# talmolab/sleap

Measured on NVIDIA H100. Metric: frames/sec (1024x1024 bottom-up UNet+PAF), higher is better.
Workload: dtype f16

## Files before the change

### sleap_b200/csrc/sb_conv_tc.cu

```cuda
#include <cuda.h>

#include <algorithm>

#include "sb_model.h"

namespace {

constexpr int TW = 16, TH = 8;
constexpr int MAX_GROUPS = 7, MAX_TAPS = 7;
constexpr size_t kMaxDynSmem = 225 * 1024;

struct TcTap { int row_off, w_tap; };
struct TcGroup { int dx, n_taps; TcTap taps[MAX_TAPS]; };

struct TcParams {
  int H, W;
  int tiles_x;
  int n_chunks, KC;
  int n_groups;
  TcGroup groups[MAX_GROUPS];
  int dy0, box_rows;
  int N, Cout;
  void* out;
  int out_f32, out_H, out_W, out_Ctot, out_coff;
// ... 689 lines not shown
    for (int bk = 0; bk < NB; ++bk) wgmma_reg_fence(acc[bk]);
    wgmma_wait<0>();
#pragma unroll
    for (int bk = 0; bk < NB; ++bk) wgmma_reg_fence(acc[bk]);
    __syncwarp();
    if (lane == 0) mbar_arrive(smem_u32(empty + s));

    const int tile = w % n_tiles, b = w / n_tiles;
    const int x0 = (tile % tiles_x) * 16, y0 = (tile / tiles_x) * (8 * BY);
#pragma unroll
    for (int bk = 0; bk < NB; ++bk)
      halo_block_epilogue<N>(P, acc[bk], smem_u32(s_bias), 0, b, y0 + 8 * (bk >> 1) + 2 * q, x0 + 8 * (bk & 1) + g, g, t, lo);
  }
}

constexpr int kWideThreads = 384;
constexpr int kWidePatchLoaders = 96;
constexpr int wide_by(int n) { return n <= 64 ? 4 : 2; }
constexpr int wide_plane(int n) { return (8 * wide_by(n) + 2) * kHaloCols * 16; }

template <int N>
__global__ void __launch_bounds__(kWideThreads, 1) k_conv_wg_hw(const __grid_constant__ CUtensorMap mapA,
                                                                const __grid_constant__ CUtensorMap mapB,
                                                                const __grid_constant__ TcParams P) {
  constexpr int BY = wide_by(N), NP = 8, PH = 8 * BY + 2, PW = kHaloCols, PLANE = wide_plane(N), SLOT = NP * PLANE;
  constexpr int WSLOT = N * 128;
  extern __shared__ __align__(1024) uint8_t smem_raw[];
  uint8_t* base = reinterpret_cast<uint8_t*>((reinterpret_cast<uintptr_t>(smem_raw) + 1023) & ~(uintptr_t)1023);
  uint8_t* wring = base;
  uint8_t* pring = wring + (size_t)P.n_b_slots * WSLOT;
// ... 419 lines not shown
  int threads;
  size_t smem;
  int max_ctas;
  int n_items;
  TcParams P;
  CUtensorMap mapA, mapB;
  TcPhases Q;
};

struct TcLaunch {
  dim3 grid;
  TcForm forms[kForms];
  int form;
};

}

struct SbConvTcPlan {
  std::vector<TcLaunch> launches;
  const void* head = nullptr;
  __half* w16 = nullptr;
  int Cout_pad = 0;
  bool pool_fused = false;
  bool out_dead = false;
  bool res_fused = false;
  std::vector<TcLaunch> plain_launches;
};

static CUtensorMapSwizzle swz_for(int KC) {
  return KC == 64 ? CU_TENSOR_MAP_SWIZZLE_128B : (KC == 32 ? CU_TENSOR_MAP_SWIZZLE_64B : CU_TENSOR_MAP_SWIZZLE_32B);
}

static bool tc_eligible(const SbModel* m, const SbOp& op) {
  if (getenv("SB_DISABLE_TC")) return false;
  if (op.kind() != SB_OPK_CONV && op.kind() != SB_OPK_TCONV) return false;
  const int Cin = op.in_C();
  if (!(Cin >= 16 && Cin % 8 == 0)) return false;
  if (op.kind() == SB_OPK_CONV && !((op.k() == 1 || op.k() == 3 || op.k() == 5 || op.k() == 7) && op.stride() == 1) &&
      !(op.k() == 1 && op.stride() == 2))
    return false;
  if (op.kind() == SB_OPK_CONV && op.explicit_pad() && (op.k() != 1 || op.pad_top() != 0 || op.pad_left() != 0)) return false;
// ... 135 lines not shown
  }
  F.n_items = P.n_tiles;
  fit_ctas(h, F, 1);
}

static bool res_fusable(const SbModel* m, size_t oi) {
  const SbOp& op = m->ops[oi];
  if (op.kind() != SB_OPK_CONV || !op.residual() || oi + 1 >= m->ops.size() || getenv("SB_DISABLE_RES_FUSION")) return false;
  const SbOp& add = m->ops[oi + 1];
  if (add.kind() != SB_OPK_ADD || !(add.flags() & SB_OPF_FUSED_ADD) || add.out_buf() != op.sum_buf() || add.out_coff() != op.sum_coff()) return false;
  const SbBuffer& rb = m->buffers[op.res_buf()];
  const SbBuffer& sb = m->buffers[op.sum_buf()];
  const SbBuffer& ob = m->buffers[op.out_buf()];
  return !rb.f32 && !sb.f32 && !ob.f32 && rb.C % 8 == 0 && op.res_coff() % 8 == 0 && sb.C % 8 == 0 && op.sum_coff() % 8 == 0 &&
         rb.H == ob.H && rb.W == ob.W && sb.H == ob.H && sb.W == ob.W && op.pool_buf() < 0 && !(op.flags() & (SB_OPF_BN | SB_OPF_RELU));
}

static CUresult encode_weights(EncodeTiledFn enc, const SbConvTcPlan* plan, int Cin, int n_wtaps, int KC, int box_n, CUtensorMap* map) {
  cuuint64_t dims[3] = {(cuuint64_t)Cin, (cuuint64_t)plan->Cout_pad, (cuuint64_t)n_wtaps};
  cuuint64_t strides[2] = {(cuuint64_t)Cin * 2, (cuuint64_t)plan->Cout_pad * Cin * 2};
  cuuint32_t box[3] = {(cuuint32_t)KC, (cuuint32_t)box_n, 1};
  cuuint32_t es[3] = {1, 1, 1};
  return enc(map, CU_TENSOR_MAP_DATA_TYPE_FLOAT16, 3, (void*)plan->w16, dims, strides, box, es, CU_TENSOR_MAP_INTERLEAVE_NONE,
             swz_for(KC), CU_TENSOR_MAP_L2_PROMOTION_L2_256B, CU_TENSOR_MAP_FLOAT_OOB_FILL_NONE);
}

static int make_launch(sb_handle_s* h, SbModel* m, const SbOp& op, SbConvTcPlan* plan, int n_groups,
                       const TcGroup* groups, int dy0, int extra_rows, int n_wtaps, int oy_mul, int oy_add,
                       int ox_mul, int ox_add, const SbTcView* view = nullptr, bool fuse_res = false,
                       std::vector<TcLaunch>* dst = nullptr) {
// ... 193 lines not shown
  }
#undef SB_HEAD_CASE
}

int sb_conv_tc_prepare(sb_handle_s* h, SbModel* m) {
  m->tc_plans.assign(m->ops.size(), nullptr);
  if (m->precision == 1) return 0;
  const bool split = m->precision == 2;
  static bool attr_set = false;
  if (!attr_set) {
    for (int f = 0; f < kForms; ++f)
      for (int kc : {16, 32, 64})
        for (int n : kWgN)
          if (const void* k = form_kernel(f, kc, n))
            SB_CUDA(h, cudaFuncSetAttribute(k, cudaFuncAttributeMaxDynamicSharedMemorySize, (int)kMaxDynSmem));
    attr_set = true;
  }
  for (size_t oi = 0; oi < m->ops.size(); ++oi) {
    const SbOp& op = m->ops[oi];
    if (!tc_eligible(m, op)) continue;
    const int Cin = op.in_C(), Cout = op.out_C(), k = op.k(), taps = k * k;
    SbConvTcPlan* plan = new SbConvTcPlan();
    int cp = (Cout + 15) / 16 * 16;
    if (cp > 256) cp = (cp + 255) / 256 * 256;
    plan->Cout_pad = cp;
    std::vector<__half> w16((size_t)taps * cp * Cin, __float2half(0.f));
    const float* w = m->weights_host.data() + op.w_off();
    for (int t = 0; t < taps; ++t)
      for (int ci = 0; ci < Cin; ++ci)
        for (int co = 0; co < Cout; ++co)
// ... 100 lines not shown
  TcParams P = F.P;
  P.skip_out = skip_out;
  dim3 grid(std::min(F.n_items * B, F.max_ctas));
  size_t smem = F.smem;
  if (L.form == 0) {
    grid = dim3(L.grid.x, L.grid.y, B);
    P.pdl_trigger = (sb_pdl_on() && smem >= 114 * 1024) ? 1 : 0;
    if (P.pdl_trigger) smem = std::max(smem, kMaxDynSmem);
  } else {
    P.batch = B;
  }
  void* args[4] = {const_cast<CUtensorMap*>(&F.mapA), const_cast<CUtensorMap*>(&F.mapB), &P, const_cast<TcPhases*>(&F.Q)};
  sb_launch_pdl(form_kernel(L.form, P.KC, P.N), grid, dim3(F.threads), smem, stream, args);
}

static int tc_launch(sb_handle_s* h, const std::vector<TcLaunch>& launches, int B, int skip_out) {
  for (const TcLaunch& L : launches) {
    launch_form(L, B, h->stream, skip_out);
    SB_CHECK_LAUNCH(h);
    if (L.form == kTconvForm) break;
  }
  return 0;
}

int sb_time_min(sb_handle_s* h, const char* what, float& best, const std::function<int()>& run) {
  cudaEvent_t e0, e1;
  SB_CUDA(h, cudaEventCreate(&e0));
  SB_CUDA(h, cudaEventCreate(&e1));
  best = 1e30f;
  int rc = 0;
// ... 51 lines not shown
    SbConvTcPlan* plan = m->tc_plans[oi];
    if (!plan || plan->launches.empty() || !plan->launches[0].forms[kTconvForm].ok) continue;
    TcLaunch& L0 = plan->launches[0];
    const int phase_form = L0.form;
    float best[2];
    for (int f = 0; f < 2; ++f) {
      L0.form = f ? kTconvForm : phase_form;
      snprintf(what, sizeof what, "op %zu, %s", oi, f ? "fused tconv" : "tconv phases");
      if (const int rc = sb_time_min(h, what, best[f], [&] { return tc_launch(h, plan->launches, m->B, 0); })) return rc;
    }
    L0.form = (force >= 0 ? force == kTconvForm : best[1] < best[0]) ? kTconvForm : phase_form;
    if (dbg)
      fprintf(stderr, "[sb_conv_tc] op %zu launches (4 tconv phases) %.1f us, fused k_tconv_wg_hw %.1f us -> %s\n", oi, best[0] * 1e3f,
              best[1] * 1e3f, L0.form == kTconvForm ? "tconv-fused" : "phases");
  }
  return 0;
}

static SbLaunchFn head_entry(const SbModel* m, const SbOp& op, const SbConvTcPlan* plan, bool log) {
  const SbBuffer& ib = m->buffers[op.in_buf()];
  const SbBuffer& ob = m->buffers[op.out_buf()];
  const HeadShape hs = head_shape(op);
  if (log && getenv("SB_DEBUG"))
    fprintf(stderr, "[sb_conv_tc] head k_head_1x1: Cin %d Cout %d NT %d KCH %d n_ring %d smem %zu\n", op.in_C(), op.out_C(), hs.nt,
            hs.kch, hs.n_ring, hs.smem);
  const void* kern = plan->head;
  const __half* in = (const __half*)ib.dev;
  const __half* w = plan->w16;
  const float* bias = op.b_off() >= 0 ? m->weights_dev + op.b_off() : nullptr;
  float* out = (float*)ob.dev;
  int in_Ctot = ib.C, in_coff = op.in_coff(), Cin = op.in_C(), out_Ctot = ob.C, out_coff = op.out_coff(), Cout = op.out_C();
  int relu = (op.flags() & SB_OPF_RELU) ? 1 : 0, n_ring = hs.n_ring;
  const size_t frame_pix = (size_t)ob.H * ob.W;
  return [=](sb_handle_s* h, const void*, int, int B) mutable {
    size_t npix = (size_t)B * frame_pix;
    void* args[] = {&in, &in_Ctot, &in_coff, &Cin, &w, &bias, &out, &out_Ctot, &out_coff, &Cout, &relu, &npix, &n_ring};
    const int grid = (int)std::min<size_t>((npix + 127) / 128, (size_t)h->sm_count * 2);
    sb_launch_pdl(kern, dim3(grid), dim3(256), hs.smem, h->stream, args);
    SB_CHECK_LAUNCH(h);
    return 0;
  };
}

SbTcEntry sb_conv_tc_entry(const SbModel* m, int op_index, bool all_stores) {
  const SbConvTcPlan* plan = m->tc_plans[op_index];
  SbTcEntry e;
  if (plan->head) {
    e.run = head_entry(m, m->ops[op_index], plan, !all_stores);
    return e;
  }
  const bool res = plan->res_fused && !all_stores;
  const int skip = plan->out_dead && !all_stores;
  const std::vector<TcLaunch>* launches = plan->res_fused && all_stores ? &plan->plain_launches : &plan->launches;
  e.run = [launches, skip](sb_handle_s* h, const void*, int, int B) { return tc_launch(h, *launches, B, skip); };
  if (plan->pool_fused || res) e.absorbs = op_index + 1;
  e.elides_out = skip || res;
  return e;
}
```

### sleap_b200/csrc/sb_entry.cu

```cuda
#include <algorithm>

#include "sb_model.h"

template <typename TI, int CIN, int COUT, int PX>
__global__ void __launch_bounds__(256) k_conv_first(const TI* __restrict__ img, int Hin, int Win, int Hnet, int Wnet,
                                                    __half* __restrict__ out, int out_Ctot, int out_coff,
                                                    const float* __restrict__ w ,
                                                    const float* __restrict__ bias, int relu, int in_is_u8, int split = 0) {
  __shared__ __align__(16) float s_w[9 * CIN * COUT];
  __shared__ float s_b[COUT];
  for (int t = threadIdx.y * 32 + threadIdx.x; t < 9 * CIN * COUT; t += 256) s_w[t] = w[t];
  for (int t = threadIdx.y * 32 + threadIdx.x; t < COUT; t += 256) s_b[t] = bias ? bias[t] : 0.f;
  __syncthreads();
  const int ox0 = (blockIdx.x * 32 + threadIdx.x) * PX, oy = blockIdx.y * 8 + threadIdx.y, b = blockIdx.z;
  if (ox0 >= Wnet || oy >= Hnet) return;
  const TI* im = img + (size_t)b * Hin * Win * CIN;
  const float sc = in_is_u8 ? (1.0f / 255.0f) : 1.0f;
  float acc[PX][COUT];
#pragma unroll
  for (int p = 0; p < PX; ++p)
#pragma unroll
    for (int c = 0; c < COUT; ++c) acc[p][c] = s_b[c];
#pragma unroll
  for (int ky = 0; ky < 3; ++ky) {
// ... 173 lines not shown
  if (cv.in_C() != ib.C || !only_reader(m, pre.out_buf(), p + 1)) return false;
  if (ib.H % 2 || ib.W % 2 || ob.H != ib.H / 2 || ob.W != ib.W / 2) return false;
  return !ob.f32 && ob.C % 8 == 0 && cv.out_coff() % 8 == 0;
}

bool conv01_fusable(const SbModel* m, int c0i) {
  if (m->precision != 0 || c0i + 1 >= (int)m->ops.size()) return false;
  const SbOp& c0 = m->ops[c0i];
  const SbOp& c1 = m->ops[c0i + 1];
  if (m->Cin != 1 || c0.in_C() != 1 || c0.out_C() != 16 || c0.k() != 3 || c0.stride() != 1 || (c0.flags() & SB_OPF_BN)) return false;
  if (c1.kind() != SB_OPK_CONV || c1.in_C() != 16 || c1.out_C() != 16 || c1.k() != 3 || c1.stride() != 1 || (c1.flags() & SB_OPF_BN)) return false;
  if (c1.in_buf() != c0.out_buf() || c1.in_coff() != c0.out_coff() || c1.pool_buf() < 0) return false;
  const SbBuffer& ob0 = m->buffers[c0.out_buf()];
  const SbBuffer& pb = m->buffers[c1.pool_buf()];
  if (ob0.f32 || pb.f32 || pb.C % 2 || c1.pool_coff() % 2 || ob0.H % 2 || ob0.W % 2) return false;
  return m->tc_plans[c0i + 1] && sb_conv_tc_entry(m, c0i + 1, false).elides_out && only_reader(m, c0.out_buf(), c0i + 1);
}


void free_view(SbEntryPlan& e) {
  if (e.view) cudaFree(e.view);
  if (e.view_bias) cudaFree(e.view_bias);
  e.view = nullptr;
  e.view_bias = nullptr;
}

int view_prepare(sb_handle_s* h, SbModel* m, int route, SbTcView& V, const std::vector<float>& w) {
  SbEntryPlan& e = m->entry;
  const size_t bytes = (size_t)m->B * e.view_H * e.view_W * 16 * sizeof(__half) + 256;
  SB_CUDA(h, cudaMalloc((void**)&e.view, bytes));
  SB_CUDA(h, cudaMemset(e.view, 0, bytes));
// ... 92 lines not shown
    } else {
      if (Cin == 1) launch_first<float, 1>(co, B, s, (const float*)frames_dev, Hin, Win, ob.H, ob.W, (__half*)ob.dev, ob.C, coff, Wt, bias, relu, 0, split);
      else launch_first<float, 3>(co, B, s, (const float*)frames_dev, Hin, Win, ob.H, ob.W, (__half*)ob.dev, ob.C, coff, Wt, bias, relu, 0, split);
    }
    SB_CHECK_LAUNCH(h);
    return 0;
  };
}

SbLaunchFn view_entry(SbModel* m) {
  const SbEntryPlan& e = m->entry;
  const int route = e.route, view_H = e.view_H, view_W = e.view_W, pre_mode = e.pre_mode;
  const int Cin = m->Cin, Hin = m->Hin, Win = m->Win;
  __half* view = e.view;
  const SbBuffer ib = m->buffers[m->ops[e.conv_op].in_buf()];
  const SbLaunchFn gemm = sb_conv_tc_entry(m, e.conv_op, false).run;
  return [=](sb_handle_s* h, const void* frames_dev, int frames_are_u8, int B) {
    const size_t total = (size_t)B * view_H * view_W;
    const int grid = (int)std::min<size_t>((total + 255) / 256, (size_t)h->sm_count * 16);
    cudaStream_t s = h->stream;
    if (route == SB_ENTRY_BUFFER_VIEW) {
      k_first_view<__half><<<grid, 256, 0, s>>>((const __half*)ib.dev, ib.H, ib.W, view_H, view_W, view, 0, total);
    } else if (route == SB_ENTRY_STEM_VIEW) {
      if (frames_are_u8)
        k_s2d_view<unsigned char><<<grid, 256, 0, s>>>((const unsigned char*)frames_dev, Hin, Win, Cin, view_H, view_W, view, 1,
                                                       total, pre_mode);
      else
        k_s2d_view<float><<<grid, 256, 0, s>>>((const float*)frames_dev, Hin, Win, Cin, view_H, view_W, view, 0, total, pre_mode);
    } else if (frames_are_u8) {
      k_first_view<unsigned char><<<grid, 256, 0, s>>>((const unsigned char*)frames_dev, Hin, Win, view_H, view_W, view, 1, total);
    } else {
// ... 50 lines not shown
      snprintf(what, sizeof what, "first layer, form %d", f);
      const int rc = sb_time_min(h, what, best[f], [&] { return cand[f](h, m->frames_dev, 1, m->B); });
      if (rc) return rc;
    }
    bool view = best[1] < best[0];
    if (const char* fv = getenv("SB_FORCE_FIRST_VIEW")) view = atoi(fv) != 0;
    if (dbg) fprintf(stderr, "[sb_conv_tc] op %d first layer: k_conv_first %.1f us, Toeplitz view + wgmma %.1f us -> %s\n", e.conv_op,
                     best[0] * 1e3f, best[1] * 1e3f, view ? "view" : "direct");
    if (!view) {
      sb_conv_tc_drop(m, e.conv_op);
      free_view(e);
      e.route = SB_ENTRY_DIRECT;
    }
  }
  if (e.conv01) {
    const SbLaunchFn conv0 = first_conv_entry(m), conv1 = sb_conv_tc_entry(m, e.conv_op + 1, false).run, fused_block = conv01_entry(e.conv01);
    float best[2];
    for (int f = 0; f < 2; ++f) {
      snprintf(what, sizeof what, "first block, fused %d", f);
      const int rc = sb_time_min(h, what, best[f], [&] {
        if (f == 1) return fused_block(h, m->frames_dev, 1, m->B);
        const int rc0 = conv0(h, m->frames_dev, 1, m->B);
        return rc0 ? rc0 : conv1(h, m->frames_dev, 1, m->B);
      });
      if (rc) return rc;
    }
    bool fused = best[1] < best[0];
    if (const char* fv = getenv("SB_FORCE_CONV01")) fused = atoi(fv) != 0;
    if (dbg) fprintf(stderr, "[sb_conv_tc] first block (B = %d): conv0 + conv1 launches %.1f us, fused k_conv01 %.1f us -> %s\n", m->B,
                     best[0] * 1e3f, best[1] * 1e3f, fused ? "fused" : "separate");
    if (fused) e.conv1_op = e.conv_op + 1;
  }
  return 0;
}

void sb_entry_build(SbModel* m, bool all_stores, std::vector<char>& taken) {
  const SbEntryPlan& e = m->entry;
  if (e.pre_op >= 0) taken[e.pre_op] = 1;
  if (e.conv_op < 0) return;
  const bool fused = e.conv1_op >= 0 && !all_stores;
  m->prog[all_stores][e.conv_op] = fused ? conv01_entry(e.conv01) : first_conv_entry(m);
  taken[e.conv_op] = 1;
  if (fused) taken[e.conv1_op] = taken[e.conv1_op + 1] = 1;
  if (e.conv01) m->buf_elided[m->ops[e.conv_op].out_buf()] = m->buf_elided[m->ops[e.conv_op + 1].out_buf()] = 1;
}

void sb_entry_release(SbModel* m) {
  free_view(m->entry);
  sb_conv01_release(m);
  m->entry = SbEntryPlan();
}
```

### sleap_b200/csrc/sb_model.cu

```cuda
#include <algorithm>

#include "sb_common.cuh"
#include "sb_kernels_direct.cuh"
#include "sb_model.h"

using namespace sbd;

namespace {

template <typename T> T* buf_ptr(const SbBuffer& b) { return (T*)b.dev; }

size_t elem_size(const SbModel* m, const SbBuffer& b) { return (b.f32 || m->precision == 1) ? 4 : 2; }

int grid_for(size_t total, int sm) {
  size_t g = (total + 255) / 256;
  size_t cap = (size_t)sm * 16;
  return (int)std::max<size_t>(1, std::min(g, cap));
}

int build_programs(sb_handle_s* h, SbModel* m);

}

void sb_models_free(sb_handle_s* h) {
// ... 297 lines not shown
    case SB_OPK_COPY:
      slot = [=](sb_handle_s* h, const void*, int, int B) {
        const size_t npix = (size_t)B * ob.H * ob.W;
        k_copy<T><<<grid_for(npix * op.in_C(), h->sm_count), 256, 0, h->stream>>>((const T*)ib.dev, ib.C, op.in_coff(), (T*)ob.dev, ob.C,
                                                                                  op.out_coff(), op.in_C(), npix);
        SB_CHECK_LAUNCH(h);
        return 0;
      };
      return 0;
    default:
      return sb_fail(h, SB_ERR_INVALID, "unknown op kind %d", op.kind());
  }
}

int build_programs(sb_handle_s* h, SbModel* m) {
  const size_t n = m->ops.size();
  m->op_kind.assign(n, 0);
  for (size_t oi = 0; oi < n; ++oi)
    if (m->ops[oi].kind() == SB_OPK_CONV || m->ops[oi].kind() == SB_OPK_TCONV) m->op_kind[oi] = m->tc_plans[oi] ? 1 : 2;
  m->buf_elided.assign(m->buffers.size(), 0);
  for (int all_stores = 0; all_stores < 2; ++all_stores) {
    m->prog[all_stores].assign(n, nullptr);
    std::vector<char> taken(n, 0);
    sb_entry_build(m, all_stores, taken);
    for (size_t oi = 0; oi < n; ++oi) {
      if (taken[oi]) continue;
      if (m->tc_plans[oi]) {
        const SbTcEntry e = sb_conv_tc_entry(m, (int)oi, all_stores);
        m->prog[all_stores][oi] = e.run;
        if (e.absorbs >= 0) taken[e.absorbs] = 1;
        if (e.elides_out) m->buf_elided[m->ops[oi].out_buf()] = 1;
        continue;
      }
      const int rc = m->precision == 1 ? op_entry_t<float>(h, m, m->ops[oi], m->prog[all_stores][oi])
                                       : op_entry_t<__half>(h, m, m->ops[oi], m->prog[all_stores][oi]);
      if (rc) return rc;
    }
  }
  return 0;
}

int run_program(sb_handle_s* h, SbModel* m, const std::vector<SbLaunchFn>& prog, const void* frames_dev, int frames_are_u8, int B) {
  cudaStream_t s = h->stream;
  for (size_t oi = 0; oi < prog.size(); ++oi) {
    if (!m->prof_events.empty()) cudaEventRecord(m->prof_events[oi], s);
    if ((int)oi == m->guard_op && h->post_pending) SB_CUDA(h, cudaStreamWaitEvent(s, h->post_done_ev, 0));
    if (prog[oi])
      if (const int rc = prog[oi](h, frames_dev, frames_are_u8, B)) return rc;
  }
  if (!m->prof_events.empty()) cudaEventRecord(m->prof_events[prog.size()], s);
  return 0;
}

}

int sb_run_ops(sb_handle_s* h, SbModel* m, const void* frames_dev, int frames_are_u8, int B, bool all_stores) {
  if (!m->configured) return sb_fail(h, SB_ERR_INVALID, "model not configured");
  if (B <= 0 || B > m->B) return sb_fail(h, SB_ERR_INVALID, "batch %d exceeds configured max %d", B, m->B);
  const bool timed = m->fwd_timing && 2 * (m->fwd_n + 1) <= (int)m->fwd_events.size();
  if (timed) cudaEventRecord(m->fwd_events[2 * m->fwd_n], h->stream);
  const int rc = run_program(h, m, m->prog[all_stores], frames_dev, frames_are_u8, B);
  if (timed) { cudaEventRecord(m->fwd_events[2 * m->fwd_n + 1], h->stream); ++m->fwd_n; }
  return rc;
}

__global__ void k_half_to_float(const __half* __restrict__ in, float* __restrict__ out, size_t n) {
  for (size_t t = (size_t)blockIdx.x * blockDim.x + threadIdx.x; t < n; t += (size_t)gridDim.x * blockDim.x)
    out[t] = __half2float(in[t]);
}

static int upload_frames(sb_handle_s* h, SbModel* m, const void* images_host, int is_u8, int B) {
  const size_t bytes = (size_t)B * m->Hin * m->Win * m->Cin * (is_u8 ? 1 : 4);
  SB_CUDA(h, cudaMemcpyAsync(m->frames_dev, images_host, bytes, cudaMemcpyHostToDevice, h->stream));
  return 0;
}

extern "C" {

int sb_model_forward(sb_handle_t h, int model_id, const void* images_host, int images_are_u8, int B,
                     int n_outputs, const int32_t* output_buffer_ids, float** out_host_ptrs) {
  SbModel* m = get_model(h, model_id);
  if (!m) return sb_fail(h, SB_ERR_INVALID, "bad model id");
  SB_CUDA(h, cudaSetDevice(h->device));
  if (!m->configured) return sb_fail(h, SB_ERR_INVALID, "model not configured");
  if (B <= 0 || B > m->B) return sb_fail(h, SB_ERR_INVALID, "bad batch");
  int rc = upload_frames(h, m, images_host, images_are_u8, B);
  if (rc) return rc;
  bool all_stores = false;
  for (int i = 0; i < n_outputs; ++i) {
    const int id = output_buffer_ids[i];
    if (id >= 0 && id < (int)m->buffers.size() && m->buf_elided[id]) all_stores = true;
  }
  if ((rc = sb_run_ops(h, m, m->frames_dev, images_are_u8, B, all_stores))) return rc;
  for (int i = 0; i < n_outputs; ++i) {
    const int id = output_buffer_ids[i];
    if (id < 0 || id >= (int)m->buffers.size()) return sb_fail(h, SB_ERR_INVALID, "bad output buffer id %d", id);
    SbBuffer& b = m->buffers[id];
    const size_t n = (size_t)B * b.H * b.W * b.C;
    if (elem_size(m, b) == 4) {
      SB_CUDA(h, cudaMemcpyAsync(out_host_ptrs[i], b.dev, n * 4, cudaMemcpyDeviceToHost, h->stream));
    } else {
      float* tmp = nullptr;
      SB_CUDA(h, cudaMalloc((void**)&tmp, n * 4));
      k_half_to_float<<<grid_for(n, h->sm_count), 256, 0, h->stream>>>((const __half*)b.dev, tmp, n);
      h->gpu_launches++;
      cudaError_t e = cudaMemcpyAsync(out_host_ptrs[i], tmp, n * 4, cudaMemcpyDeviceToHost, h->stream);
      cudaStreamSynchronize(h->stream);
      cudaFree(tmp);
// ... 559 lines not shown
```

### sleap_b200/csrc/sb_model.h

```cpp
#pragma once
#include <functional>
#include <vector>

#include "sb_common.cuh"

enum {
  SB_OPK_BUFFER = 0,
  SB_OPK_CONV = 1,
  SB_OPK_TCONV = 2,
  SB_OPK_POOL = 3,
  SB_OPK_UPSAMPLE = 4,
  SB_OPK_ADD = 5,
  SB_OPK_PREPROCESS = 6,
  SB_OPK_COPY = 7,
};
enum { SB_OPF_RELU = 1, SB_OPF_BN = 2, SB_OPF_BILINEAR = 8, SB_OPF_FUSED_POOL = 16, SB_OPF_EXPLICIT_PAD = 32,
       SB_OPF_FUSED_ADD = 64, SB_OPF_RESIDUAL = 128 };
enum { SB_PRE_PLAIN = 0, SB_PRE_IMAGENET_CAFFE = 1, SB_PRE_IMAGENET_CAFFE_GRAY = 2 };

struct SbOp {
  int32_t w[SB_OP_WORDS];
  int kind() const { return w[0]; }
  int in_buf() const { return w[1]; }
  int in_coff() const { return w[2]; }
// ... 19 lines not shown
  int res_buf() const { return w[20]; }
  int res_coff() const { return w[21]; }
  int sum_buf() const { return w[22]; }
  int sum_coff() const { return w[23]; }
  float input_scale() const { float f; memcpy(&f, &w[16], 4); return f; }
  int pad_stride() const { return w[17]; }
  int pre_mode() const { return w[19]; }
};

struct SbBuffer {
  int id = 0, stride_den = 1, C = 0, f32 = 0, is_input = 0;
  int H = 0, W = 0;
  void* dev = nullptr;
};

struct SbConvTcPlan;
struct SbConv01Plan;
struct SbTopdown;

using SbLaunchFn = std::function<int(sb_handle_s* h, const void* frames_dev, int frames_are_u8, int B)>;

enum {
  SB_ENTRY_GENERIC = 0,
  SB_ENTRY_DIRECT,
  SB_ENTRY_FRAME_VIEW,
  SB_ENTRY_BUFFER_VIEW,
  SB_ENTRY_STEM_VIEW,
};
struct SbEntryPlan {
  int route = SB_ENTRY_GENERIC;
// ... 8 lines not shown
};

struct SbModel {
  int precision = 0;
  std::vector<SbOp> ops;
  std::vector<SbBuffer> buffers;
  std::vector<float> weights_host;
  float* weights_dev = nullptr;
  void* weights_tc_dev = nullptr;
  int64_t n_weights = 0;
  bool configured = false;
  int B = 0, Hin = 0, Win = 0, Cin = 0, Hres = 0, Wres = 0, Hnet = 0, Wnet = 0;
  size_t act_bytes = 0;
  void* frames_dev = nullptr;
  std::vector<SbConvTcPlan*> tc_plans;
  std::vector<SbLaunchFn> prog[2];
  std::vector<int> op_kind;
  std::vector<char> buf_elided;
  std::vector<cudaEvent_t> prof_events;
  std::vector<cudaEvent_t> fwd_events;
  int fwd_n = 0;
  bool fwd_timing = false;
  SbPostWs ws;
  sb_bottomup_params bu{};
  std::vector<int> bu_edges;
  bool bu_configured = false;
  int guard_op = -1;
  void* frames_slot[2] = {nullptr, nullptr};
  float* stage_host[2] = {nullptr, nullptr};
  int slot_B[2] = {0, 0}, rec_B = 0;
  float* rec_host = nullptr;
// ... 5 lines not shown
  float *gpart = nullptr, *gpoints = nullptr, *gvals = nullptr, *crop_off_dev = nullptr;
  int g_rpc = 1, g_chunks = 1;
  sb_centroid_params ce{};
  bool ce_configured = false;
  bool td_configured = false;
  SbTopdown* td = nullptr;
  SbEntryPlan entry;
  SbGather gather;
  SbTracker* trk = nullptr;
  int trk_B = 0, trk_I = 0, trk_cut = -1;
  double trk_h = 1.0, trk_w = 1.0;
  double* trk_dev = nullptr;
  double* trk_host[3] = {nullptr, nullptr, nullptr};
};

int sb_run_ops(sb_handle_s* h, SbModel* m, const void* frames_dev, int frames_are_u8, int B, bool all_stores = false);

void sb_topdown_free(SbModel* m);

SbGatherDev sb_gather_dev(const SbModel* m, unsigned long long step);
void sb_gather_free(SbModel* m);
int sb_gather_queue_collect(sb_handle_s* h, SbModel* m, long long step, int B, float* host_dst, int* counts_dev, cudaStream_t s);
void sb_pipeline_slots_free(SbModel* m);

int sb_conv_tc_prepare(sb_handle_s* h, SbModel* m);
int sb_conv_tc_autotune(sb_handle_s* h, SbModel* m);
void sb_conv_tc_release(SbModel* m);
struct SbTcEntry {
  SbLaunchFn run;
  int absorbs = -1;
  bool elides_out = false;
};
SbTcEntry sb_conv_tc_entry(const SbModel* m, int op_index, bool all_stores);
struct SbTcView {
  SbBuffer in;
  SbBuffer out;
  int Cout = 0, out_coff = 0;
  int R = 0, S = 0, dy0 = 0, dx0 = 0;
  const float *bias = nullptr, *bn_scale = nullptr, *bn_shift = nullptr;
  int relu = 0;
};
int sb_conv_tc_view_prepare(sb_handle_s* h, SbModel* m, int op_index, const SbTcView& v, const std::vector<float>& w);
void sb_conv_tc_drop(SbModel* m, int op_index);
int sb_time_min(sb_handle_s* h, const char* what, float& best, const std::function<int()>& run);

int sb_entry_prepare(sb_handle_s* h, SbModel* m);
int sb_entry_autotune(sb_handle_s* h, SbModel* m);
void sb_entry_build(SbModel* m, bool all_stores, std::vector<char>& taken);
void sb_entry_release(SbModel* m);

int sb_conv01_prepare(sb_handle_s* h, SbModel* m, int conv0_op, int conv1_op);
void sb_conv01_release(SbModel* m);
int sb_conv01_launch(sb_handle_s* h, const SbConv01Plan* pl, const void* frames_dev, int frames_are_u8, int B);

bool sb_pdl_on();

inline cudaError_t sb_launch_pdl(const void* kernel, dim3 grid, dim3 block, size_t smem, cudaStream_t stream, void** args) {
  cudaLaunchConfig_t cfg = {};
  cfg.gridDim = grid; cfg.blockDim = block; cfg.dynamicSmemBytes = smem; cfg.stream = stream;
  cudaLaunchAttribute at[1];
  at[0].id = cudaLaunchAttributeProgrammaticStreamSerialization;
  at[0].val.programmaticStreamSerializationAllowed = 1;
  cfg.attrs = at; cfg.numAttrs = sb_pdl_on() ? 1 : 0;
// ... 3 lines not shown
```

Baseline: 4054.

## Fuse consecutive 3x3 conv pair into one kernel with shared-memory intermediate

Adds k_block_wg, which computes a 16->32 3x3 conv and the following 32->32 3x3 conv (with fused pool) per 16x16 tile. The first conv's output, halo included, stays in shared memory, so the intermediate activation no longer makes a global round trip and one launch is saved. The kernel recomputes the halo pixels and is only chosen when autotuning finds it faster than the separate launches. A third program variant is also introduced so the intermediate is written out only when a caller asks for that buffer.

```diff
diff --git a/sleap_b200/csrc/sb_conv_tc.cu b/sleap_b200/csrc/sb_conv_tc.cu
--- a/sleap_b200/csrc/sb_conv_tc.cu
+++ b/sleap_b200/csrc/sb_conv_tc.cu
@@ -727,6 +727,173 @@
   }
 }
 
+constexpr int kBlkIn = 20;
+constexpr int kBlkAPlane = 432 * 16;
+constexpr int kBlkASlot = 2 * kBlkAPlane;
+constexpr int kBlkMid = 18;
+constexpr int kBlkMPlane = kBlkMid * kBlkMid * 16;
+constexpr int kBlkMSlot = 4 * kBlkMPlane;
+constexpr int kBlkABlocks = 6;
+
+__global__ void __launch_bounds__(kConvThreads, 1) k_block_wg(const __grid_constant__ CUtensorMap mapWA,
+                                                              const __grid_constant__ CUtensorMap mapWB,
+                                                              const __grid_constant__ TcParams PA,
+                                                              const __grid_constant__ TcParams PB) {
+  extern __shared__ __align__(1024) uint8_t smem_raw[];
+  uint8_t* base = reinterpret_cast<uint8_t*>((reinterpret_cast<uintptr_t>(smem_raw) + 1023) & ~(uintptr_t)1023);
+  uint8_t* bank_a = base;
+  uint8_t* bank_b = bank_a + 9 * (size_t)PA.b_slot_bytes;
+  uint8_t* mid = bank_b + 9 * (size_t)PB.b_slot_bytes;
+  uint8_t* ring = mid + 2 * (size_t)kBlkMSlot;
+  const int n_slots = PA.n_a_slots;
+  uint64_t* full = reinterpret_cast<uint64_t*>(ring + (size_t)n_slots * kBlkASlot);
+  uint64_t* empty = full + n_slots;
+  uint64_t* fullB = empty + n_slots;
+  float* s_bias = reinterpret_cast<float*>(fullB + 1);
+
+  const int warp = threadIdx.x >> 5, lane = threadIdx.x & 31;
+  const int H = PB.H, W = PB.W;
+  const int tiles_x = (W + 15) / 16, n_tiles = tiles_x * ((H + 15) / 16);
+  const int n_work = n_tiles * PA.batch;
+  for (int i = threadIdx.x; i < 64; i += blockDim.x) {
+    const TcParams& P = i < 32 ? PA : PB;
+    s_bias[i] = P.bias ? P.bias[i & 31] : 0.f;
+  }
+  if (threadIdx.x == 0) {
+    for (int i = 0; i < n_slots; ++i) { mbar_init(smem_u32(full + i), 32); mbar_init(smem_u32(empty + i), 4); }
+    mbar_init(smem_u32(fullB), 1);
+    asm volatile("fence.mbarrier_init.release.cluster;" ::: "memory");
+    asm volatile("prefetch.tensormap [%0];" ::"l"(&mapWA) : "memory");
+    asm volatile("prefetch.tensormap [%0];" ::"l"(&mapWB) : "memory");
+  }
+  __syncthreads();
+
+  if (warp == kConsumerThreads / 32) {
+    if (lane == 0) {
+      mbar_expect_tx(smem_u32(fullB), (uint32_t)(9 * (PA.b_tx_bytes + PB.b_tx_bytes)));
+      for (int kx = 0; kx < 3; ++kx)
+        for (int ky = 0; ky < 3; ++ky) {
+          tma_load_3d(smem_u32(bank_a + (size_t)(kx * 3 + ky) * PA.b_slot_bytes), &mapWA, smem_u32(fullB), 0, 0, ky * 3 + kx);
+          tma_load_3d(smem_u32(bank_b + (size_t)(kx * 3 + ky) * PB.b_slot_bytes), &mapWB, smem_u32(fullB), 0, 0, ky * 3 + kx);
+        }
+    }
+    griddep_wait();
+    const __half* in = reinterpret_cast<const __half*>(PA.in);
+    for (int i = 0, w = blockIdx.x; w < n_work; ++i, w += gridDim.x) {
+      if (w + (int)gridDim.x >= n_work) griddep_launch();
+      const int s = i % n_slots;
+      mbar_wait(smem_u32(empty + s), ((i / n_slots) & 1) ^ 1);
+      const int tile = w % n_tiles, b = w / n_tiles;
+      const int xs = (tile % tiles_x) * 16 - 2, ys = (tile / tiles_x) * 16 - 2;
+      const uint32_t dst = smem_u32(ring + (size_t)s * kBlkASlot);
+      for (int e = lane; e < 2 * kBlkIn * kBlkIn; e += 32) {
+        const int pl = e & 1, p = e >> 1, y = ys + p / kBlkIn, x = xs + p % kBlkIn;
+        const bool ok = y >= 0 && y < H && x >= 0 && x < W;
+        const __half* src = ok ? in + (((size_t)b * H + y) * W + x) * PA.in_Ctot + pl * 8 : in;
+        asm volatile("cp.async.cg.shared.global [%0], [%1], 16, %2;" ::"r"(dst + (uint32_t)(pl * kBlkAPlane + p * 16)), "l"(src),
+                     "r"(ok ? 16 : 0) : "memory");
+      }
+      asm volatile("cp.async.mbarrier.arrive.noinc.shared::cta.b64 [%0];" ::"r"(smem_u32(full + s)) : "memory");
+    }
+    asm volatile("cp.async.wait_all;" ::: "memory");
+    return;
+  }
+
+  const int wg = warp >> 2, q = warp & 3, g = lane >> 2, t = lane & 3;
+  const float lo_a = PA.relu ? 0.f : -INFINITY, lo_b = PB.relu ? 0.f : -INFINITY;
+  const uint64_t desc_pa = make_desc_interleave(0, kBlkAPlane, 8 * 16);
+  const uint64_t desc_pm = make_desc_interleave(0, kBlkMPlane, kBlkMid * 16);
+  const uint64_t desc_wa = make_desc(0, PA.row_bytes, PA.layout_type), desc_wb = make_desc(0, PB.row_bytes, PB.layout_type);
+  const uint32_t wa_base = smem_u32(bank_a), wb_base = smem_u32(bank_b);
+  uint8_t* my_mid = mid + (size_t)wg * kBlkMSlot;
+  const uint32_t m_base = smem_u32(my_mid);
+  __half* out_a = reinterpret_cast<__half*>(PA.out) + PA.out_coff;
+  mbar_wait(smem_u32(fullB), 0);
+  for (int i = wg, w = blockIdx.x + wg * (int)gridDim.x; w < n_work; i += 2, w += 2 * (int)gridDim.x) {
+    const int s = i % n_slots;
+    const int tile = w % n_tiles, b = w / n_tiles;
+    const int x0 = (tile % tiles_x) * 16, y0 = (tile / tiles_x) * 16;
+    {
+      float acc[kBlkABlocks][16];
+      mbar_wait(smem_u32(full + s), (i / n_slots) & 1);
+      asm volatile("fence.proxy.async.shared::cta;" ::: "memory");
+      const uint32_t a_base = smem_u32(ring + (size_t)s * kBlkASlot);
+      wgmma_fence();
+#pragma unroll
+      for (int bk = 0; bk < kBlkABlocks; ++bk) wgmma_reg_fence(acc[bk]);
+#pragma unroll
+      for (int kx = 0; kx < 3; ++kx)
+#pragma unroll
+        for (int ky = 0; ky < 3; ++ky) {
+          const uint64_t db = desc_wa + (uint64_t)((wa_base + (uint32_t)((kx * 3 + ky) * PA.b_slot_bytes)) >> 4);
+#pragma unroll
+          for (int bk = 0; bk < kBlkABlocks; ++bk) {
+            const uint32_t a = a_base + (uint32_t)((64 * bk + ky * kBlkIn + kx) * 16);
+            wgmma_f16<32>(acc[bk], desc_pa + (uint64_t)(a >> 4), db, (kx | ky) ? 1u : 0u);
+          }
+        }
+      wgmma_commit();
+#pragma unroll
+      for (int bk = 0; bk < kBlkABlocks; ++bk) wgmma_reg_fence(acc[bk]);
+      wgmma_wait<0>();
+#pragma unroll
+      for (int bk = 0; bk < kBlkABlocks; ++bk) wgmma_reg_fence(acc[bk]);
+      __syncwarp();
+      if (lane == 0) mbar_arrive(smem_u32(empty + s));
+      asm volatile("bar.sync %0, 128;" ::"r"(2 + wg) : "memory");
+#pragma unroll
+      for (int bk = 0; bk < kBlkABlocks; ++bk) {
+        uint32_t hv[8];
+        frag_rows_f16<32>(acc[bk], smem_u32(s_bias), t, lo_a, hv);
+#pragma unroll
+        for (int r = 0; r < 2; ++r) {
+          const int p = 64 * bk + 16 * q + g + 8 * r, pr = p / kBlkIn, pc = p % kBlkIn;
+          if (pr >= kBlkMid || pc >= kBlkMid) continue;
+          const int yy = y0 - 1 + pr, xx = x0 - 1 + pc;
+          const bool inside = yy >= 0 && yy < H && xx >= 0 && xx < W;
+          const uint32_t d = m_base + (uint32_t)((pr * kBlkMid + pc) * 16 + 4 * t);
+#pragma unroll
+          for (int j = 0; j < 4; ++j)
+            asm volatile("st.shared.b32 [%0], %1;" ::"r"(d + (uint32_t)(j * kBlkMPlane)), "r"(inside ? hv[r * 4 + j] : 0u) : "memory");
+          if (!PA.skip_out && inside && pr >= 1 && pr <= 16 && pc >= 1 && pc <= 16) {
+            __half* po = out_a + (((size_t)b * H + yy) * W + xx) * PA.out_Ctot + 2 * t;
+#pragma unroll
+            for (int j = 0; j < 4; ++j) *reinterpret_cast<uint32_t*>(po + 8 * j) = hv[r * 4 + j];
+          }
+        }
+      }
+      asm volatile("fence.proxy.async.shared::cta;" ::: "memory");
+      asm volatile("bar.sync %0, 128;" ::"r"(2 + wg) : "memory");
+    }
+    float acc[4][16];
+    wgmma_fence();
+#pragma unroll
+    for (int bk = 0; bk < 4; ++bk) wgmma_reg_fence(acc[bk]);
+#pragma unroll
+    for (int kx = 0; kx < 3; ++kx)
+#pragma unroll
+      for (int ky = 0; ky < 3; ++ky)
+#pragma unroll
+        for (int k = 0; k < 2; ++k) {
+          const uint64_t db = desc_wb + (uint64_t)((wb_base + (uint32_t)((kx * 3 + ky) * PB.b_slot_bytes)) >> 4) + 2 * k;
+#pragma unroll
+          for (int bk = 0; bk < 4; ++bk) {
+            const uint32_t a = m_base + (uint32_t)(((8 * (bk >> 1) + ky) * kBlkMid + 8 * (bk & 1) + kx) * 16 + 2 * k * kBlkMPlane);
+            wgmma_f16<32>(acc[bk], desc_pm + (uint64_t)(a >> 4), db, (kx | ky | k) ? 1u : 0u);
+          }
+        }
+    wgmma_commit();
+#pragma unroll
+    for (int bk = 0; bk < 4; ++bk) wgmma_reg_fence(acc[bk]);
+    wgmma_wait<0>();
+#pragma unroll
+    for (int bk = 0; bk < 4; ++bk) wgmma_reg_fence(acc[bk]);
+#pragma unroll
+    for (int bk = 0; bk < 4; ++bk)
+      halo_block_epilogue<32>(PB, acc[bk], smem_u32(s_bias + 32), 0, b, y0 + 8 * (bk >> 1) + 2 * q, x0 + 8 * (bk & 1) + g, g, t, lo_b);
+  }
+}
+
 constexpr int kWideThreads = 384;
 constexpr int kWidePatchLoaders = 96;
 constexpr int wide_by(int n) { return n <= 64 ? 4 : 2; }
@@ -1176,6 +1343,13 @@
   int form;
 };
 
+struct TcBlock {
+  TcParams PA, PB;
+  CUtensorMap mapWA, mapWB;
+  size_t smem;
+  int max_ctas, n_items;
+};
+
 }
 
 struct SbConvTcPlan {
@@ -1187,6 +1361,8 @@
   bool out_dead = false;
   bool res_fused = false;
   std::vector<TcLaunch> plain_launches;
+  bool block_ok = false, block_fused = false;
+  TcBlock block;
 };
 
 static CUtensorMapSwizzle swz_for(int KC) {
@@ -1352,6 +1528,32 @@
   const SbBuffer& ob = m->buffers[op.out_buf()];
   return !rb.f32 && !sb.f32 && !ob.f32 && rb.C % 8 == 0 && op.res_coff() % 8 == 0 && sb.C % 8 == 0 && op.sum_coff() % 8 == 0 &&
          rb.H == ob.H && rb.W == ob.W && sb.H == ob.H && sb.W == ob.W && op.pool_buf() < 0 && !(op.flags() & (SB_OPF_BN | SB_OPF_RELU));
+}
+
+static bool block_fusable(const SbModel* m, int a) {
+  if (m->precision != 0 || a + 2 >= (int)m->ops.size() || a == m->entry.conv_op || a + 1 == m->entry.conv_op) return false;
+  const SbConvTcPlan* pa = m->tc_plans[a];
+  const SbConvTcPlan* pb = m->tc_plans[a + 1];
+  if (!pa || !pb || pa->head || pb->head || pa->launches.size() != 1 || pb->launches.size() != 1 || pa->pool_fused || pa->res_fused)
+    return false;
+  const SbOp& A = m->ops[a];
+  const SbOp& B = m->ops[a + 1];
+  if (A.kind() != SB_OPK_CONV || B.kind() != SB_OPK_CONV || A.k() != 3 || B.k() != 3 || A.residual() || B.residual()) return false;
+  if (A.in_C() != 16 || A.out_C() != 32 || B.in_C() != 32 || B.out_C() != 32) return false;
+  if (B.in_buf() != A.out_buf() || B.in_coff() != A.out_coff() || !pb->pool_fused || !pb->out_dead) return false;
+  for (const SbConvTcPlan* p : {pa, pb}) {
+    const TcLaunch& L = p->launches[0];
+    if (L.grid.y != 1 || L.forms[0].P.n_chunks != 1 || L.forms[0].P.N != 32 || !halo_shape(L.forms[0].P)) return false;
+  }
+  for (size_t j = 0; j < m->ops.size(); ++j) {
+    if ((int)j == a + 1) continue;
+    const SbOp& o = m->ops[j];
+    if (o.kind() == SB_OPK_PREPROCESS) continue;
+    if (o.in_buf() == A.out_buf() && o.in_coff() < A.out_coff() + 32 && A.out_coff() < o.in_coff() + o.in_C()) return false;
+    if (o.kind() == SB_OPK_ADD && o.in2_buf() == A.out_buf() && o.in2_coff() < A.out_coff() + 32 && A.out_coff() < o.in2_coff() + o.in_C())
+      return false;
+  }
+  return true;
 }
 
 static CUresult encode_weights(EncodeTiledFn enc, const SbConvTcPlan* plan, int Cin, int n_wtaps, int KC, int box_n, CUtensorMap* map) {
@@ -1575,6 +1777,7 @@
         for (int n : kWgN)
           if (const void* k = form_kernel(f, kc, n))
             SB_CUDA(h, cudaFuncSetAttribute(k, cudaFuncAttributeMaxDynamicSharedMemorySize, (int)kMaxDynSmem));
+    SB_CUDA(h, cudaFuncSetAttribute((const void*)k_block_wg, cudaFuncAttributeMaxDynamicSharedMemorySize, (int)kMaxDynSmem));
     attr_set = true;
   }
   for (size_t oi = 0; oi < m->ops.size(); ++oi) {
@@ -1705,6 +1908,37 @@
   sb_launch_pdl(form_kernel(L.form, P.KC, P.N), grid, dim3(F.threads), smem, stream, args);
 }
 
+static void setup_block(sb_handle_s* h, SbModel* m, int a) {
+  SbConvTcPlan* plan = m->tc_plans[a];
+  TcBlock& K = plan->block;
+  K.PA = plan->launches[0].forms[0].P;
+  K.PB = m->tc_plans[a + 1]->launches[0].forms[0].P;
+  K.mapWA = plan->launches[0].forms[0].mapB;
+  K.mapWB = m->tc_plans[a + 1]->launches[0].forms[0].mapB;
+  K.n_items = ((K.PB.W + 15) / 16) * ((K.PB.H + 15) / 16);
+  for (int ns = 8; ns >= 4 && !plan->block_ok; --ns) {
+    const size_t smem = 1024  + (size_t)9 * (K.PA.b_slot_bytes + K.PB.b_slot_bytes) + (size_t)2 * kBlkMSlot +
+                        (size_t)ns * kBlkASlot + (size_t)(2 * ns + 1) * 8 + 64 * sizeof(float);
+    if (smem <= kMaxDynSmem) { plan->block_ok = true; K.PA.n_a_slots = ns; K.smem = smem; }
+  }
+  int nb = 0;
+  if (!plan->block_ok || cudaOccupancyMaxActiveBlocksPerMultiprocessor(&nb, k_block_wg, kConvThreads, K.smem) != cudaSuccess || nb < 1) {
+    cudaGetLastError();
+    plan->block_ok = false;
+    return;
+  }
+  K.max_ctas = nb * h->sm_count;
+}
+
+static void launch_block(const TcBlock& K, int B, cudaStream_t stream, bool store_a, bool store_b) {
+  TcParams PA = K.PA, PB = K.PB;
+  PA.batch = PB.batch = B;
+  PA.skip_out = store_a ? 0 : 1;
+  PB.skip_out = store_b ? 0 : 1;
+  void* args[4] = {const_cast<CUtensorMap*>(&K.mapWA), const_cast<CUtensorMap*>(&K.mapWB), &PA, &PB};
+  sb_launch_pdl((const void*)k_block_wg, dim3(std::min(K.n_items * B, K.max_ctas)), dim3(kConvThreads), K.smem, stream, args);
+}
+
 static int tc_launch(sb_handle_s* h, const std::vector<TcLaunch>& launches, int B, int skip_out) {
   for (const TcLaunch& L : launches) {
     launch_form(L, B, h->stream, skip_out);
@@ -1786,6 +2020,32 @@
       fprintf(stderr, "[sb_conv_tc] op %zu launches (4 tconv phases) %.1f us, fused k_tconv_wg_hw %.1f us -> %s\n", oi, best[0] * 1e3f,
               best[1] * 1e3f, L0.form == kTconvForm ? "tconv-fused" : "phases");
   }
+  const char* fblk = getenv("SB_FORCE_BLOCK");
+  for (int a = 0; a + 1 < (int)m->tc_plans.size(); ++a) {
+    SbConvTcPlan* plan = m->tc_plans[a];
+    if (!block_fusable(m, a)) continue;
+    setup_block(h, m, a);
+    if (!plan->block_ok) continue;
+    const SbConvTcPlan* next = m->tc_plans[a + 1];
+    float best[2];
+    for (int f = 0; f < 2; ++f) {
+      snprintf(what, sizeof what, "op %d, %s", a, f ? "fused block" : "block launches");
+      if (const int rc = sb_time_min(h, what, best[f], [&] {
+            if (f) {
+              launch_block(plan->block, m->B, h->stream, false, false);
+              SB_CHECK_LAUNCH(h);
+              return 0;
+            }
+            const int rc0 = tc_launch(h, plan->launches, m->B, 0);
+            return rc0 ? rc0 : tc_launch(h, next->launches, m->B, 1);
+          }))
+        return rc;
+    }
+    plan->block_fused = fblk ? atoi(fblk) != 0 : best[1] < best[0];
+    if (dbg)
+      fprintf(stderr, "[sb_conv_tc] op %d block (B = %d): launches %.1f us, fused k_block_wg %.1f us -> %s\n", a, m->B, best[0] * 1e3f,
+              best[1] * 1e3f, plan->block_fused ? "block-fused" : "separate");
+  }
   return 0;
 }
 
@@ -1814,11 +2074,25 @@
   };
 }
 
-SbTcEntry sb_conv_tc_entry(const SbModel* m, int op_index, bool all_stores) {
+SbTcEntry sb_conv_tc_entry(const SbModel* m, int op_index, int program) {
   const SbConvTcPlan* plan = m->tc_plans[op_index];
+  const bool all_stores = program == SB_PROG_ALL_STORES;
   SbTcEntry e;
   if (plan->head) {
-    e.run = head_entry(m, m->ops[op_index], plan, !all_stores);
+    e.run = head_entry(m, m->ops[op_index], plan, program == SB_PROG_PRODUCTION);
+    return e;
+  }
+  if (plan->block_fused) {
+    const TcBlock* K = &plan->block;
+    const bool store_a = program != SB_PROG_PRODUCTION;
+    e.run = [K, store_a, all_stores](sb_handle_s* h, const void*, int, int B) {
+      launch_block(*K, B, h->stream, store_a, all_stores);
+      SB_CHECK_LAUNCH(h);
+      return 0;
+    };
+    e.absorbs = op_index + 2;
+    e.elides_out = !store_a;
+    e.elides_absorbed = !all_stores;
     return e;
   }
   const bool res = plan->res_fused && !all_stores;
diff --git a/sleap_b200/csrc/sb_entry.cu b/sleap_b200/csrc/sb_entry.cu
--- a/sleap_b200/csrc/sb_entry.cu
+++ b/sleap_b200/csrc/sb_entry.cu
@@ -211,7 +211,7 @@
   const SbBuffer& ob0 = m->buffers[c0.out_buf()];
   const SbBuffer& pb = m->buffers[c1.pool_buf()];
   if (ob0.f32 || pb.f32 || pb.C % 2 || c1.pool_coff() % 2 || ob0.H % 2 || ob0.W % 2) return false;
-  return m->tc_plans[c0i + 1] && sb_conv_tc_entry(m, c0i + 1, false).elides_out && only_reader(m, c0.out_buf(), c0i + 1);
+  return m->tc_plans[c0i + 1] && sb_conv_tc_entry(m, c0i + 1, SB_PROG_PRODUCTION).elides_out && only_reader(m, c0.out_buf(), c0i + 1);
 }
 
 
@@ -334,7 +334,7 @@
   const int Cin = m->Cin, Hin = m->Hin, Win = m->Win;
   __half* view = e.view;
   const SbBuffer ib = m->buffers[m->ops[e.conv_op].in_buf()];
-  const SbLaunchFn gemm = sb_conv_tc_entry(m, e.conv_op, false).run;
+  const SbLaunchFn gemm = sb_conv_tc_entry(m, e.conv_op, SB_PROG_PRODUCTION).run;
   return [=](sb_handle_s* h, const void* frames_dev, int frames_are_u8, int B) {
     const size_t total = (size_t)B * view_H * view_W;
     const int grid = (int)std::min<size_t>((total + 255) / 256, (size_t)h->sm_count * 16);
@@ -415,7 +415,7 @@
     }
   }
   if (e.conv01) {
-    const SbLaunchFn conv0 = first_conv_entry(m), conv1 = sb_conv_tc_entry(m, e.conv_op + 1, false).run, fused_block = conv01_entry(e.conv01);
+    const SbLaunchFn conv0 = first_conv_entry(m), conv1 = sb_conv_tc_entry(m, e.conv_op + 1, SB_PROG_PRODUCTION).run, fused_block = conv01_entry(e.conv01);
     float best[2];
     for (int f = 0; f < 2; ++f) {
       snprintf(what, sizeof what, "first block, fused %d", f);
@@ -435,15 +435,16 @@
   return 0;
 }
 
-void sb_entry_build(SbModel* m, bool all_stores, std::vector<char>& taken) {
+void sb_entry_build(SbModel* m, int program, std::vector<char>& taken) {
   const SbEntryPlan& e = m->entry;
   if (e.pre_op >= 0) taken[e.pre_op] = 1;
   if (e.conv_op < 0) return;
-  const bool fused = e.conv1_op >= 0 && !all_stores;
-  m->prog[all_stores][e.conv_op] = fused ? conv01_entry(e.conv01) : first_conv_entry(m);
+  const bool fused = e.conv1_op >= 0 && program != SB_PROG_ALL_STORES;
+  m->prog[program][e.conv_op] = fused ? conv01_entry(e.conv01) : first_conv_entry(m);
   taken[e.conv_op] = 1;
   if (fused) taken[e.conv1_op] = taken[e.conv1_op + 1] = 1;
-  if (e.conv01) m->buf_elided[m->ops[e.conv_op].out_buf()] = m->buf_elided[m->ops[e.conv_op + 1].out_buf()] = 1;
+  if (e.conv01)
+    m->buf_elided[m->ops[e.conv_op].out_buf()] = m->buf_elided[m->ops[e.conv_op + 1].out_buf()] = SB_PROG_ALL_STORES;
 }
 
 void sb_entry_release(SbModel* m) {
diff --git a/sleap_b200/csrc/sb_model.cu b/sleap_b200/csrc/sb_model.cu
--- a/sleap_b200/csrc/sb_model.cu
+++ b/sleap_b200/csrc/sb_model.cu
@@ -335,29 +335,37 @@
 }
 
 int build_programs(sb_handle_s* h, SbModel* m) {
-  const size_t n = m->ops.size();
+  const size_t n = m->ops.size(), nb = m->buffers.size();
   m->op_kind.assign(n, 0);
   for (size_t oi = 0; oi < n; ++oi)
     if (m->ops[oi].kind() == SB_OPK_CONV || m->ops[oi].kind() == SB_OPK_TCONV) m->op_kind[oi] = m->tc_plans[oi] ? 1 : 2;
-  m->buf_elided.assign(m->buffers.size(), 0);
-  for (int all_stores = 0; all_stores < 2; ++all_stores) {
-    m->prog[all_stores].assign(n, nullptr);
+  m->buf_elided.assign(nb, SB_PROG_PRODUCTION);
+  std::vector<char> elided[SB_N_PROGS];
+  for (int p = 0; p < SB_N_PROGS; ++p) {
+    m->prog[p].assign(n, nullptr);
+    elided[p].assign(nb, 0);
     std::vector<char> taken(n, 0);
-    sb_entry_build(m, all_stores, taken);
+    sb_entry_build(m, p, taken);
     for (size_t oi = 0; oi < n; ++oi) {
       if (taken[oi]) continue;
       if (m->tc_plans[oi]) {
-        const SbTcEntry e = sb_conv_tc_entry(m, (int)oi, all_stores);
-        m->prog[all_stores][oi] = e.run;
-        if (e.absorbs >= 0) taken[e.absorbs] = 1;
-        if (e.elides_out) m->buf_elided[m->ops[oi].out_buf()] = 1;
+        const SbTcEntry e = sb_conv_tc_entry(m, (int)oi, p);
+        m->prog[p][oi] = e.run;
+        for (int j = (int)oi + 1; j <= e.absorbs; ++j) {
+          taken[j] = 1;
+          if (e.elides_absorbed && m->ops[j].kind() == SB_OPK_CONV) elided[p][m->ops[j].out_buf()] = 1;
+        }
+        if (e.elides_out) elided[p][m->ops[oi].out_buf()] = 1;
         continue;
       }
-      const int rc = m->precision == 1 ? op_entry_t<float>(h, m, m->ops[oi], m->prog[all_stores][oi])
-                                       : op_entry_t<__half>(h, m, m->ops[oi], m->prog[all_stores][oi]);
+      const int rc = m->precision == 1 ? op_entry_t<float>(h, m, m->ops[oi], m->prog[p][oi])
+                                       : op_entry_t<__half>(h, m, m->ops[oi], m->prog[p][oi]);
       if (rc) return rc;
     }
   }
+  for (size_t b = 0; b < nb; ++b)
+    if (m->buf_elided[b] == SB_PROG_PRODUCTION && elided[SB_PROG_PRODUCTION][b])
+      m->buf_elided[b] = elided[SB_PROG_BLOCK_STORES][b] ? SB_PROG_ALL_STORES : SB_PROG_BLOCK_STORES;
   return 0;
 }
 
@@ -375,12 +383,12 @@
 
 }
 
-int sb_run_ops(sb_handle_s* h, SbModel* m, const void* frames_dev, int frames_are_u8, int B, bool all_stores) {
+int sb_run_ops(sb_handle_s* h, SbModel* m, const void* frames_dev, int frames_are_u8, int B, int program) {
   if (!m->configured) return sb_fail(h, SB_ERR_INVALID, "model not configured");
   if (B <= 0 || B > m->B) return sb_fail(h, SB_ERR_INVALID, "batch %d exceeds configured max %d", B, m->B);
   const bool timed = m->fwd_timing && 2 * (m->fwd_n + 1) <= (int)m->fwd_events.size();
   if (timed) cudaEventRecord(m->fwd_events[2 * m->fwd_n], h->stream);
-  const int rc = run_program(h, m, m->prog[all_stores], frames_dev, frames_are_u8, B);
+  const int rc = run_program(h, m, m->prog[program], frames_dev, frames_are_u8, B);
   if (timed) { cudaEventRecord(m->fwd_events[2 * m->fwd_n + 1], h->stream); ++m->fwd_n; }
   return rc;
 }
@@ -407,12 +415,13 @@
   if (B <= 0 || B > m->B) return sb_fail(h, SB_ERR_INVALID, "bad batch");
   int rc = upload_frames(h, m, images_host, images_are_u8, B);
   if (rc) return rc;
-  bool all_stores = false;
+  int program = SB_PROG_PRODUCTION;
   for (int i = 0; i < n_outputs; ++i) {
     const int id = output_buffer_ids[i];
-    if (id >= 0 && id < (int)m->buffers.size() && m->buf_elided[id]) all_stores = true;
-  }
-  if ((rc = sb_run_ops(h, m, m->frames_dev, images_are_u8, B, all_stores))) return rc;
+    if (id < 0 || id >= (int)m->buffers.size() || m->buf_elided[id] == SB_PROG_PRODUCTION) continue;
+    if (m->buf_elided[id] == SB_PROG_ALL_STORES || program == SB_PROG_PRODUCTION) program = m->buf_elided[id];
+  }
+  if ((rc = sb_run_ops(h, m, m->frames_dev, images_are_u8, B, program))) return rc;
   for (int i = 0; i < n_outputs; ++i) {
     const int id = output_buffer_ids[i];
     if (id < 0 || id >= (int)m->buffers.size()) return sb_fail(h, SB_ERR_INVALID, "bad output buffer id %d", id);
diff --git a/sleap_b200/csrc/sb_model.h b/sleap_b200/csrc/sb_model.h
--- a/sleap_b200/csrc/sb_model.h
+++ b/sleap_b200/csrc/sb_model.h
@@ -57,6 +57,8 @@
   void* dev = nullptr;
 };
 
+enum { SB_PROG_PRODUCTION = 0, SB_PROG_ALL_STORES = 1, SB_PROG_BLOCK_STORES = 2, SB_N_PROGS = 3 };
+
 struct SbConvTcPlan;
 struct SbConv01Plan;
 struct SbTopdown;
@@ -95,7 +97,7 @@
   size_t act_bytes = 0;
   void* frames_dev = nullptr;
   std::vector<SbConvTcPlan*> tc_plans;
-  std::vector<SbLaunchFn> prog[2];
+  std::vector<SbLaunchFn> prog[SB_N_PROGS];
   std::vector<int> op_kind;
   std::vector<char> buf_elided;
   std::vector<cudaEvent_t> prof_events;
@@ -131,7 +133,7 @@
   double* trk_host[3] = {nullptr, nullptr, nullptr};
 };
 
-int sb_run_ops(sb_handle_s* h, SbModel* m, const void* frames_dev, int frames_are_u8, int B, bool all_stores = false);
+int sb_run_ops(sb_handle_s* h, SbModel* m, const void* frames_dev, int frames_are_u8, int B, int program = SB_PROG_PRODUCTION);
 
 void sb_topdown_free(SbModel* m);
 
@@ -147,8 +149,9 @@
   SbLaunchFn run;
   int absorbs = -1;
   bool elides_out = false;
+  bool elides_absorbed = false;
 };
-SbTcEntry sb_conv_tc_entry(const SbModel* m, int op_index, bool all_stores);
+SbTcEntry sb_conv_tc_entry(const SbModel* m, int op_index, int program);
 struct SbTcView {
   SbBuffer in;
   SbBuffer out;
@@ -163,7 +166,7 @@
 
 int sb_entry_prepare(sb_handle_s* h, SbModel* m);
 int sb_entry_autotune(sb_handle_s* h, SbModel* m);
-void sb_entry_build(SbModel* m, bool all_stores, std::vector<char>& taken);
+void sb_entry_build(SbModel* m, int program, std::vector<char>& taken);
 void sb_entry_release(SbModel* m);
 
 int sb_conv01_prepare(sb_handle_s* h, SbModel* m, int conv0_op, int conv1_op);
```

Result: faster. 4181 (median of 6 runs) (+3.1%).
